# nolan-h-hamilton/ROCCO

Hardware: AMD Instinct MI355X
Metric: loci/sec to converged solve, hg38 50bp K=100; BED3 intervals bit-exact (higher is better)
Workload: dtype f64

## Files before the change

rocco_amd/csrc/budget.hip:

```cpp
#include "budget.h"

#include <algorithm>
#include <atomic>
#include <chrono>
#include <cmath>
#include <cstdio>
#include <cstdlib>
#include <cstring>
#include <thread>

#include "chain.h"
#include "model_chain.h"
#include "chain_fast.h"
#include "lean.h"
#include "lean_tasks.h"
#include "search.h"

namespace rocco {

namespace {

struct DevProblem {
    const double *scores = nullptr;
    const double *costs = nullptr;
// ... 1505 lines not shown
                        child.sep = ct.sep;
                        child.pool_mark = mark;
                        ls.levels.push_back(child);
                    } else {
                        ls.pool_at = mark;
                    }
                }
            }
            LeanLevel &lv = ls.levels.back();
            const int np = (int)r.lambdas.size();
            const int nt = lean_tiles(lv.m);
            if (lv.cap_points < np) {
                const int cap = std::max(np, (ls.levels.size() > 1) ? kLeanMaxPoints : 8);
                lv.bits = (unsigned *)lean_alloc(ls, (size_t)cap * (size_t)nt * kLeanThreads * sizeof(unsigned));
                lv.tile_off = (unsigned *)lean_alloc(ls, (size_t)cap * (size_t)nt * sizeof(unsigned));
                if (lv.bits == nullptr || lv.tile_off == nullptr) {
                    set_last_error("lean evaluation: level pool exhausted");
                    return ROCCO_HIP_ENOMEM;
                }
                lv.cap_points = cap;
            }
            lv.has_eval = false;
            LeanTask t = lean_task(lv.s, lv.m, p.gamma, p.qexp,
                                   LeanTaskKind::bound_stored((long long)(lv.bits - pool_words), (long long)(lv.tile_off - pool_words)), np);
            place(t, r, tasks, units);
            if (r.comp != nullptr) {
                r.mark = ls.pool_at;
                r.capacity = lv.m + 2;
                r.out_s = (double *)lean_alloc(ls, (size_t)r.capacity * sizeof(double));
                r.out_orig = (int *)lean_alloc(ls, (size_t)r.capacity * sizeof(int));
                r.sep = separator_score(r.lambdas[0], p.gamma);
                if (r.out_s != nullptr && r.out_orig != nullptr) {
                    LeanCompactTask ct;
                    ct.s = lv.s;
                    ct.orig = lv.orig;
                    ct.m = lv.m;
                    ct.n_tiles = nt;
                    ct.block_begin = post_blocks;
                    ct.bits = lv.bits;
                    ct.tile_off = lv.tile_off;
                    ct.sep = r.sep;
                    ct.out_s = r.out_s;
                    ct.out_orig = r.out_orig;
                    ct.capacity = r.capacity;
                    post.push_back(ct);
                    post_blocks += nt;
                } else {
                    ls.pool_at = r.mark;
                    r.out_s = nullptr;
                }
            }
        }
        if (env_flag("ROCCO_HIP_LEAN_BATCH", true)) {
            lean_rebatch(tasks, kLeanBatch, units);
            lean_rebatch(model_tasks, kLeanModelBatch, model_units);
        }
        lean_units += units + model_units;
        if (model_tiles + model_tiles_answered_ > 0) {
            model_tiles_last_round_ = model_tiles + model_tiles_answered_;
        }
        const int n_bound_tasks = (int)tasks.size();
        tasks.insert(tasks.end(), model_tasks.begin(), model_tasks.end());

        Layout desc;
        const size_t o_pre = desc.at(pre.size() * sizeof(LeanCompactTask));
        const size_t o_tasks = desc.at(tasks.size() * sizeof(LeanTask));
        const size_t o_points = desc.at(points.size() * sizeof(double));
        const size_t o_post = desc.at(post.size() * sizeof(LeanCompactTask));
        const size_t o_wcap = desc.at(wcap_tasks.size() * sizeof(LeanWcapTask));
        if ((rc = solver_->dev_lean_desc.reserve(desc.bytes() + 256)) != ROCCO_HIP_OK) return rc;
        if ((rc = solver_->host_lean_stage.reserve(desc.bytes() + 256)) != ROCCO_HIP_OK) return rc;
        char *h = (char *)solver_->host_lean_stage.ptr;
        char *d = (char *)solver_->dev_lean_desc.ptr;
        if (!pre.empty()) std::memcpy(h + o_pre, pre.data(), pre.size() * sizeof(LeanCompactTask));
        std::memcpy(h + o_tasks, tasks.data(), tasks.size() * sizeof(LeanTask));
        std::memcpy(h + o_points, points.data(), points.size() * sizeof(double));
        if (!post.empty()) std::memcpy(h + o_post, post.data(), post.size() * sizeof(LeanCompactTask));
        if (!wcap_tasks.empty()) std::memcpy(h + o_wcap, wcap_tasks.data(), wcap_tasks.size() * sizeof(LeanWcapTask));
        const double le1 = now_us();
        ROCCO_HIP_TRY(hipMemcpyAsync(d, h, desc.bytes(), hipMemcpyHostToDevice, stream_));
        const double le2 = now_us();
        t_lean_cpu_ += le1 - le0;
        t_lean_h2d_ += le2 - le1;
        struct Launches {
            double &acc;
            double t0;
            ~Launches() { acc += now_us() - t0; }
        } launches{t_lean_launch_, le2};
        if (!wcap_tasks.empty()) {
            if ((rc = launch_lean_wcap((const LeanWcapTask *)(d + o_wcap), (int)wcap_tasks.size(), wcap_blocks, stream_)) != ROCCO_HIP_OK) return rc;
        }

        if ((rc = reserve_round_scratch(recs, env_flag("ROCCO_HIP_LEAN_FILLS", false))) != ROCCO_HIP_OK) return rc;
        if ((rc = solver_->host_lean_back.reserve(align_up((size_t)results * sizeof(LeanResult) + 64, 256))) != ROCCO_HIP_OK) return rc;
        LeanResult *results_host = (LeanResult *)solver_->host_lean_back.ptr;
        unsigned *error_host = (unsigned *)((char *)solver_->host_lean_back.ptr + (size_t)results * sizeof(LeanResult));
        error_host[0] = 0u;
        error_host[1] = 0u;
        LeanLaunch L = round_launch((const LeanTask *)(d + o_tasks), (const double *)(d + o_points), results_host);
        unsigned *error = L.error;
        if (!pre.empty()) {
            if ((rc = launch_lean_compact((const LeanCompactTask *)(d + o_pre), (int)pre.size(), pre_blocks, error, stream_)) != ROCCO_HIP_OK) return rc;
        }
        L.n_tasks = n_bound_tasks;
        L.n_units = units;
        L.error_out = error_host;
        solver_->lean_look_dirty = 1;
        if ((rc = launch_lean_eval(L, stream_)) != ROCCO_HIP_OK) return rc;
// ... 1582 lines not shown
```

rocco_amd/csrc/chain.hip:

```cpp
#include "chain.h"

#include <cmath>

namespace rocco {

namespace {

constexpr int kDirectorWaves = 16;
constexpr int kDirectorThreads = 64 * kDirectorWaves;

__device__ __forceinline__ double snap_to_grid(double x, int qexp) { return ldexp(rint(ldexp(x, -qexp)), qexp); }

__device__ __forceinline__ int ceil_log2_exact(double x)
{
    const int e = ilogb(x);
    return (x == ldexp(1.0, e)) ? e : e + 1;
}

__device__ __forceinline__ unsigned long long align_up_dev(unsigned long long x, unsigned long long a) { return (x + a - 1) / a * a; }

__device__ __forceinline__ char *pool_alloc(const ChainArgs &A, ChainHot &H, unsigned long long bytes)
{
    const unsigned long long at = align_up_dev(H.pool_at, 256);
    if (at + bytes > H.pool_end) {
// ... 664 lines not shown
            s_batch = batch;
            A.ctl->n_tasks = (int)n_tasks;
            A.ctl->n_units = (int)units;
            A.ctl->n_pairs = (int)pairs;
            A.ctl->n_pre_tasks = (int)n_pre;
            A.ctl->n_pre_blocks = (int)pre_blocks;
            A.ctl->round = round + 1;
            A.ctl->all_done = (n_tasks == 0 && n_pre == 0) ? 1 : 0;
        }
    }
    __syncthreads();
    if (trace) trace[4] = (long long)wall_clock64();
    for (int b = wave; b < B; b += kDirectorWaves) {
        if (lane != 0) {
            continue;
        }
        ChainHot &H = sh[b];
        if (s_np[b] < 0) {
            give_up(H);
        }
        if (s_pre_idx[b] >= 0) {
            LeanCompactTask ct = s_ct[b];
            ct.block_begin = s_pre_block[b];
            A.pre[s_pre_idx[b]] = ct;
        }
        if (s_task[b] >= 0) {
            const int np = s_np[b];
            const bool pilot = (s_flex[b] == 2);
            const int qexp = H.qexp;
            LeanTask t;
            t.s = pilot ? H.scores : H.lv_s;
            t.m = pilot ? H.n : H.lv_m;
            t.c_raw = H.gamma;
            t.magic = ldexp(1.5, 52 + qexp);
            t.big = ldexp(1.0, 50 + qexp);
            t.n_tiles = s_nt[b];
            t.n_points = np;
            t.n_groups = (np + s_batch - 1) / s_batch;
            t.unit_begin = s_unit[b];
            t.point_begin = b * kLeanMaxPoints;
            t.rec_begin = s_rec[b];
            t.bits_begin = pilot ? 0 : (long long)(H.lv_bits - (const unsigned *)A.pool);
            t.off_begin = pilot ? 0 : (long long)(H.lv_tile_off - (const unsigned *)A.pool);
            t.result_begin = b * kLeanMaxPoints;
            t.tile_stride = pilot ? s_stride[b] : 1;
            t.independent = pilot ? 1 : 0;
            t.store = pilot ? 0 : 1;
            t.emap = nullptr;
            t.wcap = nullptr;
            t.clean_chunks = nullptr;
            t.cmax = 0.0;
            t.sabs = 0.0;
            t.qexp = qexp;
            t.batch = s_batch;
            A.tasks[s_task[b]] = t;
            H.kind = pilot ? 1 : 2;
            H.np = np;
        }
        ChainProb &P = A.probs[b];
        P.smin = H.smin;
        P.smax = H.smax;
        P.sabs_sum = H.sabs_sum;
        P.eps = H.eps;
        P.qexp = H.qexp;
        P.searching = H.searching;
        P.done = H.done;
        P.rounds = H.rounds;
        P.pilots = H.pilots;
        P.n_evals = H.n_evals;
        P.n_levels = H.n_levels;
        P.pad = 0;
        P.pool_at = H.pool_at;
    }
    __syncthreads();
    {
        unsigned long long *dst = reinterpret_cast<unsigned long long *>(A.hot);
        const unsigned long long *src = reinterpret_cast<const unsigned long long *>(sh);
        for (int i = threadIdx.x; i < B * kHotWords; i += kDirectorThreads) {
            dst[i] = src[i];
        }
    }
    if (trace) trace[5] = (long long)wall_clock64();
    if (A.follow != nullptr && (last != 0 || A.ctl->all_done != 0)) {
        __syncthreads();
        const unsigned long long *src = reinterpret_cast<const unsigned long long *>(A.probs);
        unsigned long long *dst = A.follow + 32;
        for (int i = threadIdx.x; i < A.follow_words; i += kDirectorThreads) {
            dst[i] = src[i];
        }
        if (threadIdx.x < (int)(sizeof(LeanRoundCtl) / 8)) {
            dst[A.follow_ctl_word + threadIdx.x] = reinterpret_cast<const unsigned long long *>(A.ctl)[threadIdx.x];
        }
        __threadfence_system();
        __syncthreads();
        if (threadIdx.x == 0) {
            __hip_atomic_store(A.follow, 1ull, __ATOMIC_RELEASE, __HIP_MEMORY_SCOPE_SYSTEM);
        }
    }
}

}

int launch_chain_director(const ChainArgs &A, int round, int last, hipStream_t stream)
{
    hipLaunchKernelGGL(chain_director_kernel, dim3(1), dim3(kDirectorThreads), 0, stream, A, round, last);
    ROCCO_HIP_TRY(hipGetLastError());
    return ROCCO_HIP_OK;
// ... 4 lines not shown
```

rocco_amd/csrc/lean.h:

```cpp
#pragma once

#include "common.h"

namespace rocco {

constexpr int kLeanChunk = 32;
constexpr int kLeanThreads = 256;
constexpr int kLeanTile = kLeanChunk * kLeanThreads;
constexpr int kLeanBatch = 8;
constexpr int kLeanMaxPoints = 64;

struct LeanTileRec {
    unsigned base;
    unsigned tail;
    unsigned cells;
    unsigned flags;
};

struct LeanTask {
    const double *s;
    long long m;
    double c_raw;
    double magic;
    double big;
    int n_tiles;
    int n_points;
    int n_groups;
    int unit_begin;
    int point_begin;
    int rec_begin;
    long long bits_begin;
    long long off_begin;
    int result_begin;
    int tile_stride;
    int independent;
    int store;
    const uint8_t *emap;
    const double *wcap;
    const unsigned *clean_chunks;
    double cmax, sabs;
    int qexp;
    int batch;
};

struct LeanResult {
    long long count;
    long long child_len;
    long long flags;
};

struct LeanRoundCtl {
    int n_tasks;
    int n_units;
    int n_pairs;
    int n_pre_tasks;
    int n_pre_blocks;
    unsigned error;
    int round;
    int all_done;
};

struct LeanLaunch {
// ... 94 lines not shown
```

rocco_amd/csrc/lean.hip:

```cpp
#include "lean.h"
#include "model_chain.h"

#include <cmath>

namespace rocco {

namespace {

constexpr int kStride = kLeanChunk + 2;
constexpr int kTileLds = kLeanThreads * kStride;
constexpr unsigned long long kSentinel = ~0ull;
constexpr unsigned kSpinLimit = 1u << 22;

struct Fn {
    double a, lo, hi;
};

__device__ __forceinline__ double clampd(double x, double lo, double hi) { return fmin(fmax(x, lo), hi); }

__device__ __forceinline__ Fn compose(const Fn &f, const Fn &g)
{
    Fn r;
    r.a = f.a + g.a;
    r.lo = clampd(f.lo + g.a, g.lo, g.hi);
// ... 5 lines not shown
{
    Fn r;
    r.a = __shfl_up(f.a, off);
    r.lo = __shfl_up(f.lo, off);
    r.hi = __shfl_up(f.hi, off);
    return r;
}

__device__ __forceinline__ unsigned long long granule_load(const unsigned long long *p)
{
    return __hip_atomic_load(p, __ATOMIC_RELAXED, __HIP_MEMORY_SCOPE_AGENT);
}

__device__ __forceinline__ void granule_store(unsigned long long *p, double v)
{
    __hip_atomic_store(p, (unsigned long long)__double_as_longlong(v), __ATOMIC_RELAXED, __HIP_MEMORY_SCOPE_AGENT);
}

__device__ __forceinline__ double granule_wait(const unsigned long long *p, unsigned *error)
{
    unsigned long long v = granule_load(p);
    unsigned spins = 0;
    while (v == kSentinel) {
        __builtin_amdgcn_s_sleep(2);
        v = granule_load(p);
        if (++spins > kSpinLimit) {
            atomicOr(error, 1u);
            return 0.0;
        }
    }
    return __longlong_as_double((long long)v);
}

template <typename First>
__device__ __forceinline__ int find_task(int n_tasks, int key, First first_of)
{
    const int lane = threadIdx.x & 63;
    int ti = 0;
    for (int base = 0; base < n_tasks; base += 64) {
        const int i = base + lane;
        const int v = (i < n_tasks) ? first_of(i) : 0x7FFFFFFF;
        const unsigned long long le = __ballot(v <= key);
        if (le == 0ull) {
            break;
        }
        ti = base + 63 - __builtin_clzll(le);
        if (le != ~0ull) {
            break;
        }
    }
    return ti;
}

template <bool RAW>
__device__ __forceinline__ void stage_tile(const double *__restrict__ s, long long m, long long base, double magic,
                                           double *lds)
{
    const int t = threadIdx.x;
    const bool aligned16 = ((reinterpret_cast<uintptr_t>(s) & 15U) == 0);
    if (aligned16 && base + kLeanTile <= m) {
        const double2 *__restrict__ src = reinterpret_cast<const double2 *>(s + base) + t;
        double2 v[16];
#pragma unroll
        for (int r = 0; r < 16; ++r) {
            v[r] = src[r * kLeanThreads];
        }
#pragma unroll
        for (int r = 0; r < 16; ++r) {
            const int e = 2 * (r * kLeanThreads + t);
            double2 w;
            w.x = RAW ? v[r].x : (v[r].x + magic) - magic;
            w.y = RAW ? v[r].y : (v[r].y + magic) - magic;
            *reinterpret_cast<double2 *>(lds + (e >> 5) * kStride + (e & 31)) = w;
        }
    } else {
#pragma unroll 4
        for (int r = 0; r < 16; ++r) {
            const int e = 2 * (r * kLeanThreads + t);
            const long long j = base + e;
            double2 v = make_double2(0.0, 0.0);
            if (j < m) v.x = s[j];
            if (j + 1 < m) v.y = s[j + 1];
            if (!RAW) {
                v.x = (v.x + magic) - magic;
                v.y = (v.y + magic) - magic;
            }
            *reinterpret_cast<double2 *>(lds + (e >> 5) * kStride + (e & 31)) = v;
        }
    }
    __syncthreads();
}

struct Scratch {
    double wave_fn[4][kLeanBatch][3];
    double tile_in[kLeanBatch];
    unsigned red[kLeanBatch][4];
    unsigned char wave_pass[4][kLeanBatch], wave_v[4][kLeanBatch];
    unsigned first_word[4][kLeanBatch];
    unsigned last_word[kLeanBatch];
    unsigned uncertain[kLeanBatch];
    int ticket;
    int pad[3];
};

template <int PB>
__device__ __forceinline__ void chunk_function(const double *__restrict__ row, const double (&x)[PB], double c,
                                               double c_first, double big, Fn (&f)[PB])
{
    double lo[PB], hi[PB], fa[PB];
#pragma unroll
    for (int p = 0; p < PB; ++p) {
        fa[p] = 0.0;
        lo[p] = -big;
        hi[p] = big;
    }
#pragma unroll 1
    for (int i0 = 0; i0 < kLeanChunk; i0 += 8) {
        double rs[8];
#pragma unroll
        for (int ii = 0; ii < 8; ii += 2) {
            const double2 v = *reinterpret_cast<const double2 *>(row + i0 + ii);
            rs[ii] = v.x;
            rs[ii + 1] = v.y;
        }
#pragma unroll
        for (int ii = 0; ii < 8; ++ii) {
            const double cc = (i0 + ii == 0) ? c_first : c;
#pragma unroll
            for (int p = 0; p < PB; ++p) {
                const double a = rs[ii] - x[p];
                fa[p] += a;
// ... 251 lines not shown
                        wacc[p] = 0.0;
                        pre[p] = false;
                    }
                }
            }
        }
    }
#pragma unroll
    for (int p = 0; p < PB; ++p) {
        tol.clear[p] = !pre[p];
        tol.tail[p] = wacc[p];
        (void)valid;
    }
}

constexpr int kZeroBytes = 16384;

__global__ __launch_bounds__(256) void lean_zero_batch_kernel(const LeanScatterTask *__restrict__ tasks, int n_tasks)
{
    const int ti = find_task(n_tasks, (int)blockIdx.x, [&](int i) { return tasks[i].zero_begin; });
    const LeanScatterTask task = tasks[ti];
    const long long at = (long long)((int)blockIdx.x - task.zero_begin) * kZeroBytes;
    uint8_t *p = task.full + at;
    const long long len = min((long long)kZeroBytes, task.n - at);
    if (len == kZeroBytes && ((reinterpret_cast<uintptr_t>(p) & 15U) == 0)) {
        uint4 *q = reinterpret_cast<uint4 *>(p);
        const uint4 z = make_uint4(0u, 0u, 0u, 0u);
#pragma unroll
        for (int r = 0; r < kZeroBytes / 16 / 256; ++r) {
            q[r * 256 + threadIdx.x] = z;
        }
    } else {
        for (long long i = threadIdx.x; i < len; i += 256) {
            p[i] = 0;
        }
    }
}

__global__ __launch_bounds__(256) void lean_scatter_batch_kernel(const LeanScatterTask *__restrict__ tasks, int n_tasks)
{
    const int ti = find_task(n_tasks, (int)blockIdx.x, [&](int i) { return tasks[i].scatter_begin; });
    const LeanScatterTask task = tasks[ti];
    const long long i = (long long)((int)blockIdx.x - task.scatter_begin) * 256 + threadIdx.x;
    if (i < task.m) {
        const int o = task.orig[i];
        if (o >= 0) {
            task.full[o] = task.level_solution[i];
        }
    }
}

template <int PB, bool MODEL>
__device__ __forceinline__ void eval_body(const LeanLaunch &L, const LeanTask &task, int tile, int p0, int np, double *lds,
                                          Scratch *sc)
{
    const int t = threadIdx.x;
    const int lane = t & 63, wave = t >> 6;
    const long long base = (long long)tile * task.tile_stride * kLeanTile;
    const bool indep = task.independent != 0;

    const double c = (task.c_raw + task.magic) - task.magic;
    const double big = task.big;
    double x[PB];
#pragma unroll
    for (int p = 0; p < PB; ++p) {
        x[p] = L.points[task.point_begin + p0 + min(p, np - 1)];
    }
    const long long j0 = base + (long long)t * kLeanChunk;
    const bool first_unclamped = (j0 == 0 || (indep && t == 0));
    const double c_first = first_unclamped ? big : c;
    const double *row = lds + t * kStride;
    LaneModel<PB> lm;
    if (MODEL) {
        const long long chunk = j0 / kLeanChunk;
        const long long last_chunk = (task.m - 1) / kLeanChunk;
        lane_model<PB>(task, (int)task.emap[min(chunk, last_chunk)], x, lm);
    }

    Fn f[PB];
    if (MODEL) {
        chunk_function_model<PB>(row, x, lm, first_unclamped, big, f);
    } else {
        chunk_function<PB>(row, x, c, c_first, big, f);
    }
    Fn inc[PB];
#pragma unroll
    for (int p = 0; p < PB; ++p) {
        inc[p] = f[p];
    }
#pragma unroll
    for (int off = 1; off < 64; off <<= 1) {
#pragma unroll
        for (int p = 0; p < PB; ++p) {
            const Fn prev = shfl_up_fn(inc[p], off);
            if (lane >= off) {
                inc[p] = compose(prev, inc[p]);
            }
        }
    }
    if (lane == 63) {
#pragma unroll
        for (int p = 0; p < PB; ++p) {
            sc->wave_fn[wave][p][0] = inc[p].a;
            sc->wave_fn[wave][p][1] = inc[p].lo;
            sc->wave_fn[wave][p][2] = inc[p].hi;
        }
    }
    __syncthreads();

    if (t < np) {
        const int p = t;
        Fn agg;
        agg.a = sc->wave_fn[0][p][0];
        agg.lo = sc->wave_fn[0][p][1];
        agg.hi = sc->wave_fn[0][p][2];
#pragma unroll
        for (int w = 1; w < 4; ++w) {
            Fn g;
            g.a = sc->wave_fn[w][p][0];
            g.lo = sc->wave_fn[w][p][1];
            g.hi = sc->wave_fn[w][p][2];
            agg = compose(agg, g);
        }
        const long long rec = (long long)task.rec_begin + (long long)(p0 + p) * task.n_tiles + tile;
        unsigned long long *mine = L.look + rec * 4;
        const bool more = (tile + 1 < task.n_tiles) && !indep;
        if (more) {
            granule_store(mine + 0, agg.lo);
            granule_store(mine + 1, agg.hi);
            if (agg.lo == agg.hi) {
                granule_store(mine + 3, agg.lo);
            }
        }
        double din = 0.0;
        if (tile > 0 && !indep) {
            const unsigned long long *prev = L.look + (rec - 1) * 4;
            const double plo = granule_wait(prev + 0, L.error);
            const double phi = granule_wait(prev + 1, L.error);
            din = (plo == phi) ? plo : granule_wait(prev + 3, L.error);
        }
        sc->tile_in[p] = din;
        if (more && agg.lo != agg.hi) {
            granule_store(mine + 3, clampd(din + agg.a, agg.lo, agg.hi));
        }
    }
    __syncthreads();

    double din[PB];
#pragma unroll
    for (int p = 0; p < PB; ++p) {
        Fn e = shfl_up_fn(inc[p], 1);
        if (lane == 0) {
            e.a = 0.0;
            e.lo = -big;
            e.hi = big;
        }
        double v = sc->tile_in[min(p, np - 1)];
        for (int w = 0; w < wave; ++w) {
            v = clampd(v + sc->wave_fn[w][p][0], sc->wave_fn[w][p][1], sc->wave_fn[w][p][2]);
        }
        din[p] = clampd(v + e.a, e.lo, e.hi);
    }
    const bool edge_tile = (base + kLeanTile >= task.m);
    const int valid = (int)max(0LL, min((long long)kLeanChunk, task.m - j0));
    const int last = (task.m - 1 >= j0 && task.m - 1 < j0 + kLeanChunk) ? (int)(task.m - 1 - j0) : -1;
    unsigned one[PB], nz[PB];
    if (MODEL) {
        LaneTolerance<PB> tol;
        if (edge_tile) {
            chunk_classes_model<PB, true>(row, x, lm, first_unclamped, big, din, valid, last, one, nz, tol);
        } else {
            chunk_classes_model<PB, false>(row, x, lm, first_unclamped, big, din, valid, last, one, nz, tol);
        }
        const double wcap = *task.wcap;
        const double q_step = ldexp(1.0, task.qexp);
        const int e_gamma = tie_exponent(task.c_raw);
#pragma unroll
        for (int p = 0; p < PB; ++p) {
            double extra = 0.0;
            const int e_lam = tie_exponent(x[p]);
            if (e_lam + kModelMapBias >= 0 && e_lam + kModelMapBias < 128) {
                const unsigned chunks = task.clean_chunks[e_lam + kModelMapBias];
                const double hb = ldexp(1.0, e_lam + 2 - 53);
                extra += (chunks != 0u) ? (double)chunks * (double)kLeanChunk * (4.0 * hb + q_step) + 9.0 * hb + 2.0 * q_step : 0.0;
            }
            if (e_gamma != e_lam && e_gamma + kModelMapBias >= 0 && e_gamma + kModelMapBias < 128) {
                const unsigned chunks = task.clean_chunks[e_gamma + kModelMapBias];
                const double hb = ldexp(1.0, e_gamma + 2 - 53);
                extra += (chunks != 0u) ? (double)chunks * (double)kLeanChunk * (4.0 * hb + q_step) + 9.0 * hb + 2.0 * q_step : 0.0;
            }
            const double wave_in = (base == 0 && wave == 0) ? 0.0 : wcap + extra;
            bool cl = tol.clear[p];
            double tl = tol.tail[p];
#pragma unroll
            for (int off = 1; off < 64; off <<= 1) {
                const int pc = __shfl_up((int)cl, off);
                const double pt = __shfl_up(tl, off);
                if (lane >= off) {
                    tl = cl ? tl : pt + tl;
                    cl = cl || (pc != 0);
                }
            }
            int ec = __shfl_up((int)cl, 1);
            double et = __shfl_up(tl, 1);
            if (lane == 0) {
                ec = 0;
                et = 0.0;
            }
            const double w_in = ec ? et : wave_in + et;
            unsigned why = tol.bad[p];
// ... 591 lines not shown
    const int total = tasks[n_tasks - 1].block_begin + tasks[n_tasks - 1].n_tiles;
    for (int block = blockIdx.x; block < total; block += gridDim.x) {
        const int ti = find_task(n_tasks, block, [&](int i) { return tasks[i].block_begin; });
        const LeanWriteTask task = tasks[ti];
        const int tile = block - task.block_begin;
        const int t = threadIdx.x;
        const unsigned entering = task.entering[tile];
        const unsigned z = (entering != 0u ? task.word1 : task.word0)[(long long)tile * kLeanThreads + t];
        const long long j0 = (long long)tile * kLeanTile + (long long)t * kLeanChunk;
        if (j0 + kLeanChunk <= task.m && ((reinterpret_cast<uintptr_t>(task.solution + j0) & 15u) == 0u)) {
            uint4 lo, hi;
            unsigned *w = reinterpret_cast<unsigned *>(&lo);
#pragma unroll
            for (int q = 0; q < 4; ++q) {
                unsigned v = 0u;
#pragma unroll
                for (int b = 0; b < 4; ++b) {
                    v |= ((z >> (31 - (4 * q + b))) & 1u) << (8 * b);
                }
                w[q] = v;
            }
            w = reinterpret_cast<unsigned *>(&hi);
#pragma unroll
            for (int q = 0; q < 4; ++q) {
                unsigned v = 0u;
#pragma unroll
                for (int b = 0; b < 4; ++b) {
                    v |= ((z >> (31 - (16 + 4 * q + b))) & 1u) << (8 * b);
                }
                w[q] = v;
            }
            *reinterpret_cast<uint4 *>(task.solution + j0) = lo;
            *reinterpret_cast<uint4 *>(task.solution + j0 + 16) = hi;
        } else {
            for (int b = 0; b < kLeanChunk && j0 + b < task.m; ++b) {
                task.solution[j0 + b] = (uint8_t)((z >> (31 - b)) & 1u);
            }
        }
    }
}

__global__ __launch_bounds__(256) void lean_scatter_kernel(const uint8_t *__restrict__ level, const int *__restrict__ orig,
                                                           long long m, uint8_t *__restrict__ full)
{
    const long long i = (long long)blockIdx.x * 256 + threadIdx.x;
    if (i < m) {
        const int o = orig[i];
        if (o >= 0) {
            full[o] = level[i];
        }
    }
}

__global__ __launch_bounds__(kLeanThreads, 2) void lean_eval_kernel(LeanLaunch L)
{
    extern __shared__ __attribute__((aligned(16))) double smem[];
    double *lds = smem;
    Scratch *sc = reinterpret_cast<Scratch *>(smem + kTileLds);
    const int t = threadIdx.x;
    if (t == 0) {
        sc->ticket = (int)(atomicAdd(L.ticket, 1u) + 1u);
    }
    if (t < kLeanBatch * 4) {
        (&sc->red[0][0])[t] = 0u;
    }
    __syncthreads();
    const int ticket = sc->ticket;
    if (ticket >= L.n_units) {
        return;
    }
    const int ti = find_task(L.n_tasks, ticket, [&](int i) { return L.tasks[i].unit_begin; });
    const LeanTask task = L.tasks[ti];
    const int unit = ticket - task.unit_begin;
    const int tile = unit / task.n_groups, group = unit % task.n_groups;
    const int p0 = group * task.batch;
    const int np = min(task.batch, task.n_points - p0);
    stage_tile<false>(task.s, task.m, (long long)tile * task.tile_stride * kLeanTile, task.magic, lds);
    if (np > 4) {
        eval_body<8, false>(L, task, tile, p0, np, lds, sc);
    } else if (np > 2) {
        eval_body<4, false>(L, task, tile, p0, np, lds, sc);
    } else if (np > 1) {
        eval_body<2, false>(L, task, tile, p0, np, lds, sc);
    } else {
        eval_body<1, false>(L, task, tile, p0, np, lds, sc);
    }
}

__global__ __launch_bounds__(kLeanThreads, 2) void lean_eval_chain_kernel(LeanLaunch L)
{
    extern __shared__ __attribute__((aligned(16))) double smem[];
    double *lds = smem;
    Scratch *sc = reinterpret_cast<Scratch *>(smem + kTileLds);
    const int t = threadIdx.x;
    const int n_units = L.ctl->n_units, n_tasks = L.ctl->n_tasks;
    if (n_units <= 0) {
        return;
    }
    for (;;) {
        if (t == 0) {
            sc->ticket = (int)(atomicAdd(L.ticket, 1u) + 1u);
        }
        if (t < kLeanBatch * 4) {
            (&sc->red[0][0])[t] = 0u;
        }
        __syncthreads();
        const int ticket = sc->ticket;
        if (ticket >= n_units) {
            return;
        }
        const int ti = find_task(n_tasks, ticket, [&](int i) { return L.tasks[i].unit_begin; });
        const LeanTask task = L.tasks[ti];
        const int unit = ticket - task.unit_begin;
        const int tile = unit / task.n_groups, group = unit % task.n_groups;
        const int p0 = group * task.batch;
        const int np = min(task.batch, task.n_points - p0);
        stage_tile<false>(task.s, task.m, (long long)tile * task.tile_stride * kLeanTile, task.magic, lds);
        if (np > 4) {
            eval_body<8, false>(L, task, tile, p0, np, lds, sc);
        } else if (np > 2) {
            eval_body<4, false>(L, task, tile, p0, np, lds, sc);
        } else if (np > 1) {
            eval_body<2, false>(L, task, tile, p0, np, lds, sc);
        } else {
            eval_body<1, false>(L, task, tile, p0, np, lds, sc);
        }
        __syncthreads();
    }
}

__global__ __launch_bounds__(kLeanThreads, 2) void lean_model_kernel(LeanLaunch L)
{
    extern __shared__ __attribute__((aligned(16))) double smem[];
    double *lds = smem;
    Scratch *sc = reinterpret_cast<Scratch *>(smem + kTileLds);
    const int t = threadIdx.x;
    if (t == 0) {
        sc->ticket = (int)(atomicAdd(L.ticket, 1u) + 1u);
    }
    if (t < kLeanBatch * 4) {
        (&sc->red[0][0])[t] = 0u;
    }
    if (t < kLeanBatch) {
        sc->uncertain[t] = 0u;
    }
    __syncthreads();
    const int ticket = sc->ticket;
    if (ticket >= L.n_units) {
        return;
    }
    const int ti = find_task(L.n_tasks, ticket, [&](int i) { return L.tasks[i].unit_begin; });
    const LeanTask task = L.tasks[ti];
    const int unit = ticket - task.unit_begin;
    const int tile = unit / task.n_groups, group = unit % task.n_groups;
    const int p0 = group * task.batch;
    const int np = min(task.batch, task.n_points - p0);
    stage_tile<true>(task.s, task.m, (long long)tile * kLeanTile, task.magic, lds);
    if (np > 2) {
        eval_body<4, true>(L, task, tile, p0, np, lds, sc);
    } else if (np > 1) {
        eval_body<2, true>(L, task, tile, p0, np, lds, sc);
    } else {
        eval_body<1, true>(L, task, tile, p0, np, lds, sc);
    }
}

__global__ __launch_bounds__(kLeanThreads, 2) void lean_model_chain_kernel(LeanLaunch L)
{
    extern __shared__ __attribute__((aligned(16))) double smem[];
    double *lds = smem;
    Scratch *sc = reinterpret_cast<Scratch *>(smem + kTileLds);
    const int t = threadIdx.x;
    const int n_units = L.ctl->n_units, n_tasks = L.ctl->n_tasks;
    if (n_units <= 0) {
        return;
    }
    for (;;) {
        if (t == 0) {
            sc->ticket = (int)(atomicAdd(L.ticket, 1u) + 1u);
        }
        if (t < kLeanBatch * 4) {
            (&sc->red[0][0])[t] = 0u;
        }
        if (t < kLeanBatch) {
            sc->uncertain[t] = 0u;
        }
        __syncthreads();
        const int ticket = sc->ticket;
        if (ticket >= n_units) {
            return;
        }
        const int ti = find_task(n_tasks, ticket, [&](int i) { return L.tasks[i].unit_begin; });
        const LeanTask task = L.tasks[ti];
        const int unit = ticket - task.unit_begin;
        const int tile = unit / task.n_groups, group = unit % task.n_groups;
        const int p0 = group * task.batch;
        const int np = min(task.batch, task.n_points - p0);
        stage_tile<true>(task.s, task.m, (long long)tile * kLeanTile, task.magic, lds);
        if (np > 2) {
            eval_body<4, true>(L, task, tile, p0, np, lds, sc);
        } else if (np > 1) {
            eval_body<2, true>(L, task, tile, p0, np, lds, sc);
        } else {
            eval_body<1, true>(L, task, tile, p0, np, lds, sc);
        }
        __syncthreads();
    }
}

__global__ __launch_bounds__(kLeanThreads) void lean_wcap_count_kernel(const LeanWcapTask *__restrict__ tasks, int n_tasks)
{
    __shared__ unsigned steps[128], ties[128], clean[128];
    __shared__ double magic_u[kLeanThreads], half_u[kLeanThreads];
    const int ti = find_task(n_tasks, (int)blockIdx.x, [&](int i) { return tasks[i].block_begin; });
    const LeanWcapTask task = tasks[ti];
    const int t = threadIdx.x;
    if (t < 128) {
        steps[t] = 0u;
        ties[t] = 0u;
        clean[t] = 0u;
    }
    __syncthreads();
    const long long base = (long long)((int)blockIdx.x - task.block_begin) * kLeanTile;
    const long long n_chunks = (task.m + kLeanChunk - 1) / kLeanChunk;
    const long long chunk = base / kLeanChunk + t;
    int my_bin = 0;
    magic_u[t] = 0.0;
    half_u[t] = 0.0;
    if (chunk < n_chunks) {
        const int code = task.emap[chunk];
        int e = (code & 0x7F) - kModelMapBias;
        const bool code_hz = (code & 0x80) != 0;
        if (code_hz) {
            e = max(e, task.e_floor);
        }
        my_bin = min(max(e + kModelMapBias, 0), 127);
        if (code_hz || e - 52 < task.qexp) {
            atomicAdd(&steps[my_bin], (unsigned)kLeanChunk);
        } else {
            magic_u[t] = ldexp(1.5, e);
            half_u[t] = ldexp(1.0, e - 53);
            atomicAdd(&clean[my_bin], 1u);
        }
    }
    __syncthreads();
#pragma unroll 4
    for (int r = 0; r < kLeanChunk; ++r) {
        const int el = r * kLeanThreads + t;
        const long long j = base + el;
        const int c = el / kLeanChunk;
        if (j < task.m && half_u[c] != 0.0) {
            const double x = task.s[j];
            const double su = (x + magic_u[c]) - magic_u[c];
            if (fabs(x - su) == half_u[c]) {
                atomicAdd(&ties[min(max(ilogb(half_u[c]) + 53 + kModelMapBias, 0), 127)], 1u);
            }
        }
    }
    __syncthreads();
    if (t < 128) {
        if (steps[t] != 0u) {
            atomicAdd(&task.counters[t], steps[t]);
        }
        if (ties[t] != 0u) {
            atomicAdd(&task.counters[128 + t], ties[t]);
        }
        if (clean[t] != 0u) {
            atomicAdd(&task.counters[256 + t], clean[t]);
        }
    }
}

__global__ __launch_bounds__(128) void lean_wcap_sum_kernel(const LeanWcapTask *__restrict__ tasks, int n_tasks)
{
    __shared__ unsigned st_s[128], tn_s[128];
    const int ti = blockIdx.x;
    if (ti >= n_tasks) {
        return;
    }
    const LeanWcapTask task = tasks[ti];
    const int b = threadIdx.x;
    st_s[b] = task.counters[b];
    tn_s[b] = task.counters[128 + b];
    task.clean_chunks[b] = task.counters[256 + b];
    task.counters[b] = 0u;
    task.counters[128 + b] = 0u;
    task.counters[256 + b] = 0u;
    __syncthreads();
    if (b == 0) {
        const double q = ldexp(1.0, task.qexp);
        double sum = 0.0, base = 0.0;
        for (int k = 0; k < 128; ++k) {
            const int e = k - kModelMapBias;
            const unsigned st = st_s[k], tn = tn_s[k];
            if (st != 0u) {
                const double hb = ldexp(1.0, e + 2 - 53);
                sum += (double)st * (4.0 * hb + q);
                base = 9.0 * hb + 2.0 * q;
            }
            if (tn != 0u) {
                sum += (double)tn * ldexp(1.0, e - 52);
            }
        }
        task.wcap[0] = sum + base;
    }
}

int launch_eval_all(const LeanLaunch &L, hipStream_t stream)
{
    static bool configured = false;
    const size_t lds = (size_t)kTileLds * sizeof(double) + sizeof(Scratch);
    if (!configured) {
        ROCCO_HIP_TRY(hipFuncSetAttribute(reinterpret_cast<const void *>(lean_eval_kernel),
                                          hipFuncAttributeMaxDynamicSharedMemorySize, (int)lds));
        configured = true;
    }
    hipLaunchKernelGGL(lean_eval_kernel, dim3((unsigned)L.n_units), dim3(kLeanThreads), lds, stream, L);
    return ROCCO_HIP_OK;
}

}

int launch_lean_eval(const LeanLaunch &L, hipStream_t stream)
{
    if (L.n_units <= 0) {
        return ROCCO_HIP_OK;
    }
    int rc = launch_eval_all(L, stream);
    if (rc != ROCCO_HIP_OK) {
        return rc;
    }
    ROCCO_HIP_TRY(hipGetLastError());
    return ROCCO_HIP_OK;
}

int launch_lean_eval_chain(const LeanLaunch &L, int grid, hipStream_t stream)
{
    static bool configured = false;
    const size_t lds = (size_t)kTileLds * sizeof(double) + sizeof(Scratch);
    if (!configured) {
        ROCCO_HIP_TRY(hipFuncSetAttribute(reinterpret_cast<const void *>(lean_eval_chain_kernel),
                                          hipFuncAttributeMaxDynamicSharedMemorySize, (int)lds));
        configured = true;
    }
    hipLaunchKernelGGL(lean_eval_chain_kernel, dim3((unsigned)grid), dim3(kLeanThreads), lds, stream, L);
    return ROCCO_HIP_OK;
}

int launch_lean_finish_chain(const LeanLaunch &L, int grid, hipStream_t stream)
{
    hipLaunchKernelGGL(lean_finish_chain_kernel, dim3((unsigned)grid), dim3(64), 0, stream, L);
    return ROCCO_HIP_OK;
}

int launch_lean_compact_chain(const LeanCompactTask *tasks_dev, LeanRoundCtl *ctl, int grid, hipStream_t stream)
{
    hipLaunchKernelGGL(lean_compact_chain_kernel, dim3((unsigned)grid), dim3(kLeanThreads), 0, stream, tasks_dev, ctl);
    return ROCCO_HIP_OK;
}

int launch_lean_model(const LeanLaunch &L, hipStream_t stream)
{
    if (L.n_units <= 0) {
        return ROCCO_HIP_OK;
    }
    static bool configured = false;
    const size_t lds = (size_t)kTileLds * sizeof(double) + sizeof(Scratch);
    if (!configured) {
        ROCCO_HIP_TRY(hipFuncSetAttribute(reinterpret_cast<const void *>(lean_model_kernel),
                                          hipFuncAttributeMaxDynamicSharedMemorySize, (int)lds));
        configured = true;
    }
    hipLaunchKernelGGL(lean_model_kernel, dim3((unsigned)L.n_units), dim3(kLeanThreads), lds, stream, L);
    ROCCO_HIP_TRY(hipGetLastError());
    return ROCCO_HIP_OK;
}

int launch_lean_model_chain(const LeanLaunch &L, int grid, hipStream_t stream)
{
    static bool configured = false;
    const size_t lds = (size_t)kTileLds * sizeof(double) + sizeof(Scratch);
    if (!configured) {
        ROCCO_HIP_TRY(hipFuncSetAttribute(reinterpret_cast<const void *>(lean_model_chain_kernel),
                                          hipFuncAttributeMaxDynamicSharedMemorySize, (int)lds));
        configured = true;
    }
    hipLaunchKernelGGL(lean_model_chain_kernel, dim3((unsigned)grid), dim3(kLeanThreads), lds, stream, L);
    return ROCCO_HIP_OK;
}

int launch_lean_map(const LeanLaunch &L, const LeanMapOut &out, hipStream_t stream)
{
    if (L.n_units <= 0) {
        return ROCCO_HIP_OK;
    }
    static bool configured = false;
    const size_t lds = (size_t)kTileLds * sizeof(double) + sizeof(Scratch);
    if (!configured) {
// ... 86 lines not shown
```

rocco_amd/csrc/lean_tasks.h:

```cpp
#pragma once

#include <cmath>
#include <vector>

#include "model_chain.h"

namespace rocco {

inline int lean_tiles(size_t n) { return (int)((n + kLeanTile - 1) / kLeanTile); }

struct LeanTaskKind {
    int batch = kLeanBatch;
    int store = 0;
    long long bits_begin = 0, off_begin = 0;
    int tile_stride = 1, independent = 0;
    const uint8_t *emap = nullptr;
    const double *wcap = nullptr;
    const unsigned *clean_chunks = nullptr;
    double cmax = 0.0, sabs = 0.0;

    static LeanTaskKind bound_stored(long long bits_begin, long long off_begin)
    {
        LeanTaskKind k;
        k.store = 1;
        k.bits_begin = bits_begin;
        k.off_begin = off_begin;
        return k;
    }
    static LeanTaskKind pilot(int stride)
    {
        LeanTaskKind k;
        k.tile_stride = stride;
        k.independent = 1;
        return k;
    }
    static LeanTaskKind model(const uint8_t *emap, const double *wcap, const unsigned *clean_chunks, double cmax, double sabs)
    {
        LeanTaskKind k;
        k.batch = kLeanModelBatch;
        k.emap = emap;
        k.wcap = wcap;
        k.clean_chunks = clean_chunks;
        k.cmax = cmax;
        k.sabs = sabs;
        return k;
    }
    static LeanTaskKind map()
    {
        LeanTaskKind k;
        k.batch = 1;
        return k;
    }
};

inline LeanTask lean_task(const double *s, long long m, double gamma, int qexp, const LeanTaskKind &k, int n_points)
{
    LeanTask t = {};
    t.s = s;
    t.m = m;
    t.c_raw = gamma;
    t.magic = std::ldexp(1.5, 52 + qexp);
    t.big = std::ldexp(1.0, 50 + qexp);
    t.n_tiles = (lean_tiles((size_t)m) + k.tile_stride - 1) / k.tile_stride;
    t.n_points = n_points;
    t.n_groups = (n_points + k.batch - 1) / k.batch;
    t.bits_begin = k.bits_begin;
    t.off_begin = k.off_begin;
    t.tile_stride = k.tile_stride;
    t.independent = k.independent;
    t.store = k.store;
    t.emap = k.emap;
    t.wcap = k.wcap;
    t.clean_chunks = k.clean_chunks;
    t.cmax = k.cmax;
    t.sabs = k.sabs;
    t.qexp = qexp;
    t.batch = k.batch;
    return t;
}

struct LeanWcapSlot {
    double *wcap;
    unsigned *counters;
    unsigned *clean_chunks;
};

inline LeanWcapSlot lean_wcap_slot(void *base, size_t n_problems, size_t problem)
{
    LeanWcapSlot slot;
    slot.wcap = (double *)base + problem;
    slot.counters = (unsigned *)((char *)base + align_up(n_problems * sizeof(double), 256)) + 512 * problem;
    slot.clean_chunks = slot.counters + 384;
    return slot;
}

inline LeanWcapTask lean_wcap_task(const uint8_t *emap, const double *s, long long m, int qexp, double cmax, double sabs,
                                   const LeanWcapSlot &slot, int block_begin)
{
    LeanWcapTask wt;
    wt.emap = emap;
    wt.s = s;
    wt.m = m;
    wt.qexp = qexp;
    wt.e_floor = std::ilogb(2.0 * cmax + 2.0 * sabs + (sabs + 2.0) + 2.0);
    wt.counters = slot.counters;
    wt.clean_chunks = slot.clean_chunks;
    wt.wcap = slot.wcap;
    wt.block_begin = block_begin;
    wt.pad = 0;
    return wt;
}

inline void lean_rebatch(std::vector<LeanTask> &ts, int full, int &total_units)
{
    for (int b = 2; b < full; b *= 2) {
        long long u = 0;
        for (const LeanTask &t : ts) {
            u += (long long)t.n_tiles * ((t.n_points + b - 1) / b);
        }
        if (u <= 512) {
            int at = 0;
            for (LeanTask &t : ts) {
                t.batch = b;
                t.n_groups = (t.n_points + b - 1) / b;
                t.unit_begin = at;
                at += t.n_tiles * t.n_groups;
            }
            total_units = at;
            return;
        }
    }
}

struct ModelChainLayout {
    size_t tasks, walk, wcap, up_bytes;
    size_t state, points, results, ctl, globals, writes, n_writes, entering, bits, dev_bytes;
    size_t report, n_points, finals, facts, follow_bytes;
};

inline ModelChainLayout model_chain_layout(size_t B, size_t n_wcap, int rounds, long long cap_pairs)
{
    ModelChainLayout m;
    Layout dev;
    m.tasks = dev.at(B * sizeof(LeanTask));
    m.walk = dev.at(B * sizeof(ModelChainWalk));
    m.wcap = dev.at(n_wcap * sizeof(LeanWcapTask));
    dev.end_upload();
    m.up_bytes = dev.uploaded;
    m.state = dev.at(B * sizeof(ModelChainState));
    m.points = dev.at(B * kLeanMaxPoints * sizeof(double));
    m.results = dev.at(B * kLeanMaxPoints * sizeof(LeanResult));
    m.ctl = dev.at(sizeof(LeanRoundCtl));
    m.globals = dev.at(3 * sizeof(int));
    m.writes = dev.at(B * sizeof(LeanWriteTask));
    m.n_writes = dev.at(sizeof(int));
    m.entering = dev.at((size_t)rounds * (size_t)cap_pairs * sizeof(unsigned));
    m.bits = dev.at((size_t)rounds * (size_t)cap_pairs * 2 * 256 * sizeof(unsigned));
    m.dev_bytes = dev.bytes();
    Layout follow;
    m.report = follow.at(sizeof(ModelChainReport));
    m.n_points = follow.at((size_t)rounds * B * sizeof(int));
    m.finals = follow.at(B * sizeof(ModelChainFinal));
    m.facts = follow.at((size_t)rounds * B * kLeanMaxPoints * sizeof(ModelChainFact));
    m.follow_bytes = follow.bytes();
    return m;
}

}
```

Measured before the change: 5.690 billion.

## Split lean eval workgroups into two teams sharing one staged tile

Lean eval kernels now launch 512-thread workgroups made of two 256-thread teams. Each team evaluates a different subset of search points against the same LDS-staged score tile, with its own scratch area. The per-team point batch is halved so each unit still covers up to eight points, and the batching helpers account for the team count. The goal is to share tile staging across more points and cut per-point register pressure. The cost is larger workgroups, doubled scratch LDS, and idle teams when a unit has few points.

Result: faster. 5.786 billion (median of 4 runs) (+1.7%).

```diff
diff --git a/rocco_amd/csrc/budget.hip b/rocco_amd/csrc/budget.hip
--- a/rocco_amd/csrc/budget.hip
+++ b/rocco_amd/csrc/budget.hip
@@ -1581,8 +1581,8 @@
             }
         }
         if (env_flag("ROCCO_HIP_LEAN_BATCH", true)) {
-            lean_rebatch(tasks, kLeanBatch, units);
-            lean_rebatch(model_tasks, kLeanModelBatch, model_units);
+            lean_rebatch(tasks, kLeanBatch, kLeanTeams, units);
+            lean_rebatch(model_tasks, kLeanModelBatch, 1, model_units);
         }
         lean_units += units + model_units;
         if (model_tiles + model_tiles_answered_ > 0) {
diff --git a/rocco_amd/csrc/chain.hip b/rocco_amd/csrc/chain.hip
--- a/rocco_amd/csrc/chain.hip
+++ b/rocco_amd/csrc/chain.hip
@@ -740,7 +740,7 @@
             t.cmax = 0.0;
             t.sabs = 0.0;
             t.qexp = qexp;
-            t.batch = s_batch;
+            t.batch = lean_team_batch(s_batch, np);
             A.tasks[s_task[b]] = t;
             H.kind = pilot ? 1 : 2;
             H.np = np;
diff --git a/rocco_amd/csrc/lean.h b/rocco_amd/csrc/lean.h
--- a/rocco_amd/csrc/lean.h
+++ b/rocco_amd/csrc/lean.h
@@ -8,6 +8,17 @@
 constexpr int kLeanThreads = 256;
 constexpr int kLeanTile = kLeanChunk * kLeanThreads;
 constexpr int kLeanBatch = 8;
+constexpr int kLeanTeams = 2;
+constexpr int kLeanEvalThreads = kLeanThreads * kLeanTeams;
+constexpr int kLeanTeamBatch = kLeanBatch / kLeanTeams;
+constexpr int lean_team_batch(int per_workgroup, int n_points)
+{
+    int b = 1;
+    while (kLeanTeams * b < per_workgroup && kLeanTeams * b < n_points) {
+        b *= 2;
+    }
+    return b;
+}
 constexpr int kLeanMaxPoints = 64;
 
 struct LeanTileRec {
diff --git a/rocco_amd/csrc/lean.hip b/rocco_amd/csrc/lean.hip
--- a/rocco_amd/csrc/lean.hip
+++ b/rocco_amd/csrc/lean.hip
@@ -81,22 +81,23 @@
     return ti;
 }
 
-template <bool RAW>
+template <bool RAW, int NT = kLeanThreads>
 __device__ __forceinline__ void stage_tile(const double *__restrict__ s, long long m, long long base, double magic,
                                            double *lds)
 {
+    constexpr int kLoads = kLeanTile / (2 * NT);
     const int t = threadIdx.x;
     const bool aligned16 = ((reinterpret_cast<uintptr_t>(s) & 15U) == 0);
     if (aligned16 && base + kLeanTile <= m) {
         const double2 *__restrict__ src = reinterpret_cast<const double2 *>(s + base) + t;
-        double2 v[16];
-#pragma unroll
-        for (int r = 0; r < 16; ++r) {
-            v[r] = src[r * kLeanThreads];
-        }
-#pragma unroll
-        for (int r = 0; r < 16; ++r) {
-            const int e = 2 * (r * kLeanThreads + t);
+        double2 v[kLoads];
+#pragma unroll
+        for (int r = 0; r < kLoads; ++r) {
+            v[r] = src[r * NT];
+        }
+#pragma unroll
+        for (int r = 0; r < kLoads; ++r) {
+            const int e = 2 * (r * NT + t);
             double2 w;
             w.x = RAW ? v[r].x : (v[r].x + magic) - magic;
             w.y = RAW ? v[r].y : (v[r].y + magic) - magic;
@@ -104,8 +105,8 @@
         }
     } else {
 #pragma unroll 4
-        for (int r = 0; r < 16; ++r) {
-            const int e = 2 * (r * kLeanThreads + t);
+        for (int r = 0; r < kLoads; ++r) {
+            const int e = 2 * (r * NT + t);
             const long long j = base + e;
             double2 v = make_double2(0.0, 0.0);
             if (j < m) v.x = s[j];
@@ -463,9 +464,8 @@
 
 template <int PB, bool MODEL>
 __device__ __forceinline__ void eval_body(const LeanLaunch &L, const LeanTask &task, int tile, int p0, int np, double *lds,
-                                          Scratch *sc)
-{
-    const int t = threadIdx.x;
+                                          Scratch *sc, int t)
+{
     const int lane = t & 63, wave = t >> 6;
     const long long base = (long long)tile * task.tile_stride * kLeanTile;
     const bool indep = task.independent != 0;
@@ -475,7 +475,7 @@
     double x[PB];
 #pragma unroll
     for (int p = 0; p < PB; ++p) {
-        x[p] = L.points[task.point_begin + p0 + min(p, np - 1)];
+        x[p] = L.points[task.point_begin + p0 + max(min(p, np - 1), 0)];
     }
     const long long j0 = base + (long long)t * kLeanChunk;
     const bool first_unclamped = (j0 == 0 || (indep && t == 0));
@@ -566,7 +566,7 @@
             e.lo = -big;
             e.hi = big;
         }
-        double v = sc->tile_in[min(p, np - 1)];
+        double v = sc->tile_in[max(min(p, np - 1), 0)];
         for (int w = 0; w < wave; ++w) {
             v = clampd(v + sc->wave_fn[w][p][0], sc->wave_fn[w][p][1], sc->wave_fn[w][p][2]);
         }
@@ -1264,81 +1264,82 @@
     }
 }
 
-__global__ __launch_bounds__(kLeanThreads, 2) void lean_eval_kernel(LeanLaunch L)
+struct TeamUnit {
+    int tile;
+    int p0, np;
+    int lead;
+};
+
+__device__ __forceinline__ TeamUnit team_unit(const LeanTask &task, int ticket, int team)
+{
+    TeamUnit u;
+    const int unit = ticket - task.unit_begin;
+    u.tile = unit / task.n_groups;
+    const int first = (unit % task.n_groups) * kLeanTeams * task.batch;
+    u.lead = min(task.batch, task.n_points - first);
+    u.p0 = first + team * task.batch;
+    u.np = max(0, min(task.batch, task.n_points - u.p0));
+    if (u.np == 0) {
+        u.p0 = 0;
+    }
+    return u;
+}
+
+__device__ __forceinline__ void eval_team(const LeanLaunch &L, const LeanTask &task, const TeamUnit &u, double *lds, Scratch *sc,
+                                          int t)
+{
+    if (u.lead > 2) {
+        eval_body<4, false>(L, task, u.tile, u.p0, u.np, lds, sc, t);
+    } else if (u.lead > 1) {
+        eval_body<2, false>(L, task, u.tile, u.p0, u.np, lds, sc, t);
+    } else {
+        eval_body<1, false>(L, task, u.tile, u.p0, u.np, lds, sc, t);
+    }
+}
+
+__device__ __forceinline__ void eval_tickets(const LeanLaunch &L, int n_units, int n_tasks, bool persistent)
 {
     extern __shared__ __attribute__((aligned(16))) double smem[];
     double *lds = smem;
-    Scratch *sc = reinterpret_cast<Scratch *>(smem + kTileLds);
-    const int t = threadIdx.x;
-    if (t == 0) {
-        sc->ticket = (int)(atomicAdd(L.ticket, 1u) + 1u);
-    }
-    if (t < kLeanBatch * 4) {
-        (&sc->red[0][0])[t] = 0u;
-    }
-    __syncthreads();
-    const int ticket = sc->ticket;
-    if (ticket >= L.n_units) {
-        return;
-    }
-    const int ti = find_task(L.n_tasks, ticket, [&](int i) { return L.tasks[i].unit_begin; });
-    const LeanTask task = L.tasks[ti];
-    const int unit = ticket - task.unit_begin;
-    const int tile = unit / task.n_groups, group = unit % task.n_groups;
-    const int p0 = group * task.batch;
-    const int np = min(task.batch, task.n_points - p0);
-    stage_tile<false>(task.s, task.m, (long long)tile * task.tile_stride * kLeanTile, task.magic, lds);
-    if (np > 4) {
-        eval_body<8, false>(L, task, tile, p0, np, lds, sc);
-    } else if (np > 2) {
-        eval_body<4, false>(L, task, tile, p0, np, lds, sc);
-    } else if (np > 1) {
-        eval_body<2, false>(L, task, tile, p0, np, lds, sc);
-    } else {
-        eval_body<1, false>(L, task, tile, p0, np, lds, sc);
-    }
-}
-
-__global__ __launch_bounds__(kLeanThreads, 2) void lean_eval_chain_kernel(LeanLaunch L)
-{
-    extern __shared__ __attribute__((aligned(16))) double smem[];
-    double *lds = smem;
-    Scratch *sc = reinterpret_cast<Scratch *>(smem + kTileLds);
-    const int t = threadIdx.x;
+    Scratch *teams = reinterpret_cast<Scratch *>(smem + kTileLds);
+    const int team = threadIdx.x / kLeanThreads, t = threadIdx.x % kLeanThreads;
+    Scratch *sc = teams + team;
+    for (;;) {
+        if (threadIdx.x == 0) {
+            teams->ticket = (int)(atomicAdd(L.ticket, 1u) + 1u);
+        }
+        if (t < kLeanBatch * 4) {
+            (&sc->red[0][0])[t] = 0u;
+        }
+        __syncthreads();
+        const int ticket = teams->ticket;
+        if (ticket >= n_units) {
+            return;
+        }
+        const int ti = find_task(n_tasks, ticket, [&](int i) { return L.tasks[i].unit_begin; });
+        const LeanTask task = L.tasks[ti];
+        const TeamUnit u = team_unit(task, ticket, team);
+        stage_tile<false, kLeanEvalThreads>(task.s, task.m, (long long)u.tile * task.tile_stride * kLeanTile, task.magic, lds);
+        eval_team(L, task, u, lds, sc, t);
+        if (!persistent) {
+            return;
+        }
+        __syncthreads();
+    }
+}
+
+__global__ __launch_bounds__(kLeanEvalThreads, 4) void lean_eval_kernel(LeanLaunch L)
+{
+    eval_tickets(L, L.n_units, L.n_tasks, L.ctl != nullptr);
+}
+
+__global__ __launch_bounds__(kLeanEvalThreads, 4) void lean_eval_chain_kernel(LeanLaunch L)
+{
     const int n_units = L.ctl->n_units, n_tasks = L.ctl->n_tasks;
     if (n_units <= 0) {
         return;
     }
-    for (;;) {
-        if (t == 0) {
-            sc->ticket = (int)(atomicAdd(L.ticket, 1u) + 1u);
-        }
-        if (t < kLeanBatch * 4) {
-            (&sc->red[0][0])[t] = 0u;
-        }
-        __syncthreads();
-        const int ticket = sc->ticket;
-        if (ticket >= n_units) {
-            return;
-        }
-        const int ti = find_task(n_tasks, ticket, [&](int i) { return L.tasks[i].unit_begin; });
-        const LeanTask task = L.tasks[ti];
-        const int unit = ticket - task.unit_begin;
-        const int tile = unit / task.n_groups, group = unit % task.n_groups;
-        const int p0 = group * task.batch;
-        const int np = min(task.batch, task.n_points - p0);
-        stage_tile<false>(task.s, task.m, (long long)tile * task.tile_stride * kLeanTile, task.magic, lds);
-        if (np > 4) {
-            eval_body<8, false>(L, task, tile, p0, np, lds, sc);
-        } else if (np > 2) {
-            eval_body<4, false>(L, task, tile, p0, np, lds, sc);
-        } else if (np > 1) {
-            eval_body<2, false>(L, task, tile, p0, np, lds, sc);
-        } else {
-            eval_body<1, false>(L, task, tile, p0, np, lds, sc);
-        }
-        __syncthreads();
-    }
+    eval_tickets(L, n_units, n_tasks, true);
 }
 
 __global__ __launch_bounds__(kLeanThreads, 2) void lean_model_kernel(LeanLaunch L)
@@ -1369,11 +1370,11 @@
     const int np = min(task.batch, task.n_points - p0);
     stage_tile<true>(task.s, task.m, (long long)tile * kLeanTile, task.magic, lds);
     if (np > 2) {
-        eval_body<4, true>(L, task, tile, p0, np, lds, sc);
+        eval_body<4, true>(L, task, tile, p0, np, lds, sc, t);
     } else if (np > 1) {
-        eval_body<2, true>(L, task, tile, p0, np, lds, sc);
+        eval_body<2, true>(L, task, tile, p0, np, lds, sc, t);
     } else {
-        eval_body<1, true>(L, task, tile, p0, np, lds, sc);
+        eval_body<1, true>(L, task, tile, p0, np, lds, sc, t);
     }
 }
 
@@ -1410,11 +1411,11 @@
         const int np = min(task.batch, task.n_points - p0);
         stage_tile<true>(task.s, task.m, (long long)tile * kLeanTile, task.magic, lds);
         if (np > 2) {
-            eval_body<4, true>(L, task, tile, p0, np, lds, sc);
+            eval_body<4, true>(L, task, tile, p0, np, lds, sc, t);
         } else if (np > 1) {
-            eval_body<2, true>(L, task, tile, p0, np, lds, sc);
+            eval_body<2, true>(L, task, tile, p0, np, lds, sc, t);
         } else {
-            eval_body<1, true>(L, task, tile, p0, np, lds, sc);
+            eval_body<1, true>(L, task, tile, p0, np, lds, sc, t);
         }
         __syncthreads();
     }
@@ -1521,13 +1522,13 @@
 int launch_eval_all(const LeanLaunch &L, hipStream_t stream)
 {
     static bool configured = false;
-    const size_t lds = (size_t)kTileLds * sizeof(double) + sizeof(Scratch);
+    const size_t lds = (size_t)kTileLds * sizeof(double) + kLeanTeams * sizeof(Scratch);
     if (!configured) {
         ROCCO_HIP_TRY(hipFuncSetAttribute(reinterpret_cast<const void *>(lean_eval_kernel),
                                           hipFuncAttributeMaxDynamicSharedMemorySize, (int)lds));
         configured = true;
     }
-    hipLaunchKernelGGL(lean_eval_kernel, dim3((unsigned)L.n_units), dim3(kLeanThreads), lds, stream, L);
+    hipLaunchKernelGGL(lean_eval_kernel, dim3((unsigned)L.n_units), dim3(kLeanEvalThreads), lds, stream, L);
     return ROCCO_HIP_OK;
 }
 
@@ -1549,13 +1550,13 @@
 int launch_lean_eval_chain(const LeanLaunch &L, int grid, hipStream_t stream)
 {
     static bool configured = false;
-    const size_t lds = (size_t)kTileLds * sizeof(double) + sizeof(Scratch);
+    const size_t lds = (size_t)kTileLds * sizeof(double) + kLeanTeams * sizeof(Scratch);
     if (!configured) {
         ROCCO_HIP_TRY(hipFuncSetAttribute(reinterpret_cast<const void *>(lean_eval_chain_kernel),
                                           hipFuncAttributeMaxDynamicSharedMemorySize, (int)lds));
         configured = true;
     }
-    hipLaunchKernelGGL(lean_eval_chain_kernel, dim3((unsigned)grid), dim3(kLeanThreads), lds, stream, L);
+    hipLaunchKernelGGL(lean_eval_chain_kernel, dim3((unsigned)grid), dim3(kLeanEvalThreads), lds, stream, L);
     return ROCCO_HIP_OK;
 }
 
diff --git a/rocco_amd/csrc/lean_tasks.h b/rocco_amd/csrc/lean_tasks.h
--- a/rocco_amd/csrc/lean_tasks.h
+++ b/rocco_amd/csrc/lean_tasks.h
@@ -1,5 +1,6 @@
 #pragma once
 
+#include <algorithm>
 #include <cmath>
 #include <vector>
 
@@ -10,7 +11,8 @@
 inline int lean_tiles(size_t n) { return (int)((n + kLeanTile - 1) / kLeanTile); }
 
 struct LeanTaskKind {
-    int batch = kLeanBatch;
+    int batch = kLeanTeamBatch;
+    int teams = kLeanTeams;
     int store = 0;
     long long bits_begin = 0, off_begin = 0;
     int tile_stride = 1, independent = 0;
@@ -38,6 +40,7 @@
     {
         LeanTaskKind k;
         k.batch = kLeanModelBatch;
+        k.teams = 1;
         k.emap = emap;
         k.wcap = wcap;
         k.clean_chunks = clean_chunks;
@@ -49,6 +52,7 @@
     {
         LeanTaskKind k;
         k.batch = 1;
+        k.teams = 1;
         return k;
     }
 };
@@ -63,7 +67,7 @@
     t.big = std::ldexp(1.0, 50 + qexp);
     t.n_tiles = (lean_tiles((size_t)m) + k.tile_stride - 1) / k.tile_stride;
     t.n_points = n_points;
-    t.n_groups = (n_points + k.batch - 1) / k.batch;
+    t.n_groups = (n_points + k.batch * k.teams - 1) / (k.batch * k.teams);
     t.bits_begin = k.bits_begin;
     t.off_begin = k.off_begin;
     t.tile_stride = k.tile_stride;
@@ -75,7 +79,7 @@
     t.cmax = k.cmax;
     t.sabs = k.sabs;
     t.qexp = qexp;
-    t.batch = k.batch;
+    t.batch = (k.teams > 1) ? lean_team_batch(k.batch * k.teams, n_points) : k.batch;
     return t;
 }
 
@@ -111,9 +115,9 @@
     return wt;
 }
 
-inline void lean_rebatch(std::vector<LeanTask> &ts, int full, int &total_units)
+inline void lean_rebatch(std::vector<LeanTask> &ts, int full, int teams, int &total_units)
 {
-    for (int b = 2; b < full; b *= 2) {
+    for (int b = std::max(2, teams); b < full; b *= 2) {
         long long u = 0;
         for (const LeanTask &t : ts) {
             u += (long long)t.n_tiles * ((t.n_points + b - 1) / b);
@@ -121,7 +125,7 @@
         if (u <= 512) {
             int at = 0;
             for (LeanTask &t : ts) {
-                t.batch = b;
+                t.batch = (teams > 1) ? lean_team_batch(b, t.n_points) : b;
                 t.n_groups = (t.n_points + b - 1) / b;
                 t.unit_begin = at;
                 at += t.n_tiles * t.n_groups;
```
